# Lacadame/DiffSci

Hardware: AMD Instinct MI355X
Metric: samples/sec (50-step Karras Heun), PUNetG 64ch 128x128 (higher is better)
Workload: dtype f32 (3x3 convs: fp16 hi+lo split, 3 fp16 MFMA products, fp32 accumulate); 1 GPU; PUNetG 64-base-ch, 1x128x128 fields, batch 64 per GPU, 50-step Heun deterministic sampler (99 network evaluations); global_batch=64, parallelism=dp1 (batch shards, all-gather of samples), world_size=1, backend=none (one process), hipgraph=True

## Files before the change

diffsci_amd/_native.py:

```python
import ctypes
import os
from ctypes import POINTER, Structure, c_char_p, c_float, c_int, c_longlong, c_size_t, c_uint32, c_uint64, c_void_p

_HERE = os.path.dirname(os.path.abspath(__file__))
LIB_PATH = os.environ.get("DIFFSCI_HIP_LIB") or os.path.join(_HERE, "_lib", "libdiffsci_hip.so")

ABI_VERSION = 4
DS_IN_NETWORK, DS_IN_SCORE, DS_IN_DRIFT, DS_IN_FLOW = 0, 1, 2, 3
DS_LOAD_PLAIN, DS_LOAD_MAXPOOL2, DS_LOAD_UPSAMPLE2, DS_LOAD_AVGPOOL2 = 0, 1, 2, 3
DS_PAD_CIRCULAR = 16
DS_PAD_ZERO_H, DS_PAD_ZERO_W, DS_PAD_ZERO_D = 64, 128, 0x10000
DS_RES1_UPSAMPLED = 32
DS_PC_RAW, DS_PC_IMAGES = 1, 2
DS_SI_BLEND, DS_SI_RENOISE = 1, 2
DS_DDPM_CLASSICAL, DS_DDPM_GENERALIZED, DS_DDPM_FORWARD = 0, 1, 2
DS_DDPM_NOISE_NONE, DS_DDPM_NOISE_EPS, DS_DDPM_NOISE_PHILOX = 0, 4, 8


class EvalCoef(Structure):
    _fields_ = [("c_out", c_float), ("c_skip", c_float), ("sigma_sq", c_float),
                ("neg_mult", c_float), ("neg_lang", c_float), ("guidance", c_float),
                ("one_minus_guidance", c_float), ("input_kind", c_int), ("stochastic", c_int),
                ("scaled", c_int), ("scale", c_float), ("scale_mult", c_float), ("next_scale", c_float), ("xin_copies", c_int),
                ("nonfinite", c_void_p)]
# ... 64 lines not shown
    "ds_inorm_silu_images_supported": (c_int, [c_int, c_int]),
    "ds_inorm_silu_images": (c_int, [_P, _P, _P, _P, c_int, c_int, c_int, c_int, c_float, c_int, _P]),
    "ds_conv2d_h3_img": (c_int, [_P, _P, _P, c_int, _P, _P, c_int, _P, _P, c_int, c_int, c_int, c_int, c_int, c_int, _P, _P, _P]),
    "ds_gnorm1_apply_images": (c_int, [_P, _P, _P, _P, _P, _P, _P, c_int, c_int, c_int, c_int, c_int, c_int, c_int, _P]),
    "ds_volume_stat_tiles": (c_int, [c_int, c_size_t]),
    "ds_volume_to_slices_act": (c_int, [_P, _P, _P, c_int, c_int, c_int, c_size_t, c_int, _P]),
    "ds_wrap_pad_slices": (c_int, [_P, c_int, c_int, c_int, c_size_t, _P]),
    "ds_slices_to_volume_stats": (c_int, [_P, _P, _P, _P, _P, c_int, c_int, c_int, c_size_t, c_int, _P]),
    "ds_slice_tables": (c_int, [_P, _P, _P, _P, c_int, c_int, c_int, c_int, c_longlong, c_float, c_int, c_int, _P]),
    "ds_avgpool3d": (c_int, [_P, _P, c_int, c_int, c_int, c_int, _P]),
    "ds_upsample3d": (c_int, [_P, _P, c_int, c_int, c_int, c_int, _P]),
    "ds_avgpool3d_f": (c_int, [_P, _P, c_int, c_int, c_int, c_int, c_int, _P]),
    "ds_upsample_f": (c_int, [_P, _P, c_int, c_int, c_int, c_int, c_int, c_int, _P]),
    "ds_maxpool_f": (c_int, [_P, _P, c_int, c_int, c_int, c_int, c_int, c_int, _P]),
    "ds_cornerpool_f": (c_int, [_P, _P, _P, _P, c_int, c_int, c_int, c_int, c_int, c_int, c_int, c_int, c_int, _P]),
    "ds_conv1x1_h3_packed_bytes": (c_size_t, [c_int, c_int]),
    "ds_conv1x1_h3_pack_weights": (c_int, [_P, _P, c_int, c_int, c_int, _P]),
    "ds_conv1x1_h3": (c_int, [_P, _P, _P, c_int, _P, _P, c_int, _P, _P, c_int, c_int, c_int, c_int, c_int, c_int, _P, _P, _P, c_int, _P]),
    "ds_attention": (c_int, [_P, _P, c_int, c_int, c_int, _P]),
    "ds_attention_generic": (c_int, [_P, _P, c_int, c_int, c_int, _P]),
    "ds_attention_h3": (c_int, [_P, _P, c_int, c_int, c_int, _P, _P, _P]),
    "ds_attention_h3_workspace_bytes": (c_size_t, [c_int, c_int, c_int]),
    "ds_attention_h3_ws": (c_int, [_P, _P, _P, c_int, c_int, c_int, _P, _P, _P]),
    "ds_attention_h3_heads_workspace_bytes": (c_size_t, [c_int, c_int, c_int, c_int]),
    "ds_attention_h3_heads": (c_int, [_P, _P, _P, c_int, c_int, c_int, c_int, _P, _P, _P]),
    "ds_attention_heads_generic": (c_int, [_P, _P, c_int, c_int, c_int, c_int, _P]),
    "ds_token_l2_normalize": (c_int, [_P, c_int, c_int, c_int, c_int, c_int, c_float, c_float, _P]),
    "ds_linear": (c_int, [_P, _P, _P, _P, c_int, c_int, c_int, c_int, _P]),
    "ds_fourier_features": (c_int, [_P, _P, _P, _P, c_int, c_int, c_int, _P]),
    "ds_fourier_channels": (c_int, [_P, _P, _P, c_int, c_int, c_int, c_size_t, _P]),
    "ds_gnorm1_workspace_bytes": (c_size_t, [c_int]),
    "ds_gnorm1_stats": (c_int, [_P, _P, _P, c_int, c_int, c_int, c_float, c_int, _P]),
    "ds_groupnorm_stats": (c_int, [_P, _P, _P, c_int, c_int, c_int, c_int, c_float, _P]),
    "ds_groupnorm_apply": (c_int, [_P, _P, _P, _P, _P, c_int, c_int, c_int, c_int, c_int, _P, _P]),
    "ds_groupnorm_stats_tiles": (c_int, [_P, _P, c_int, c_int, c_int, c_int, c_longlong, c_float, _P]),
    "ds_groupnorm_table": (c_int, [_P, _P, _P, _P, _P, c_int, c_int, c_int, c_int, c_longlong, c_float, _P]),
    "ds_gnorm1_apply": (c_int, [_P, _P, _P, _P, _P, _P, _P, c_int, c_int, c_int, c_int, c_int, c_int, c_int, _P]),
    "ds_gnorm1_apply_poolf": (c_int, [_P, _P, _P, _P, _P, _P, _P, c_int, c_int, c_int, c_int, c_int, c_int, c_int, _P]),
    "ds_concat2": (c_int, [_P, _P, _P, c_int, c_size_t, c_size_t, _P]),
    "ds_add_act": (c_int, [_P, _P, _P, c_int, c_int, c_int, c_int, _P]),
    "ds_mask_blend": (c_int, [_P, _P, _P, _P, c_size_t, c_int, _P]),
    "ds_axpby": (c_int, [_P, _P, c_float, _P, c_float, c_size_t, _P]),
    "ds_div_scalar": (c_int, [_P, _P, c_float, c_size_t, _P]),
    "ds_batchnorm_eval": (c_int, [_P, _P, _P, _P, _P, _P, c_float, c_float, c_int, c_int, c_int, c_int, c_size_t, _P]),
    "ds_lerp_stack": (c_int, [_P, _P, _P, c_int, c_size_t, _P]),
    "ds_add": (c_int, [_P, _P, _P, c_size_t, _P]),
# ... 67 lines not shown
```

diffsci_amd/csrc/ds_attn3h.hip:

```cpp
#include <cstdlib>

#include "ds_common.h"
#include "ds_conv_epilogue.h"
#include "ds_h3_common.h"

namespace {

using ds::f32x4;
using ds::wave_max;
using ds_epi::f32x16;
using ds_h3::f16x8;
using ds_h3::split2;
using ds_h3::u32x4;
typedef unsigned u32x2 __attribute__((ext_vector_type(2)));

constexpr int NT = 256;
constexpr int KB = 32;
constexpr float RESCALE_T = 8.0f;

constexpr float LOG2E = 1.44269504088896341f;

__device__ __forceinline__ f16x8 as_f16x8(u32x4 v) { return __builtin_bit_cast(f16x8, v); }

template <int ET, bool IMG, bool MH>
__global__ __launch_bounds__(NT) void k_attn3h(float* out, const float* __restrict__ qkv, const u32x4* __restrict__ kimg,
                                               const u32x4* __restrict__ vimg, int L, int heads, int nb, float scale, float thr,
                                               const unsigned* in_amax, unsigned* out_amax) {
  constexpr int E = 32 * ET;
  constexpr int NDG = E / 8;
  constexpr int NS = E / 16;
  constexpr int KITEMS = NDG * KB;
  constexpr int KI = (KITEMS + NT - 1) / NT;
  constexpr int VITEMS = E * 4;
  constexpr int VI = (VITEMS + NT - 1) / NT;
  extern __shared__ __attribute__((aligned(16))) unsigned char smem[];
  constexpr int KVEC = 2 * NDG * KB;
  constexpr int VVEC = 2 * 4 * E;
  u32x4* Kbuf = reinterpret_cast<u32x4*>(smem);
  u32x4* Vbuf = Kbuf + 2 * KVEC;
  const int tid = threadIdx.x, lane = tid & 63;
  const int wv = __builtin_amdgcn_readfirstlane(tid >> 6);
  const int li = lane & 31, lh = lane >> 5;
  unsigned qblk, b_u;
  {
    const unsigned nx = gridDim.x;
    const unsigned id = blockIdx.x + nx * blockIdx.y;
    const unsigned total = nx * gridDim.y;
    const unsigned per = total >> 3, rem = total & 7u;
    const unsigned xcd = id & 7u, k = id >> 3;
    const unsigned logical = xcd * per + (xcd < rem ? xcd : rem) + k;
    qblk = logical % nx;
    b_u = logical / nx;
  }
  const int row = (int)b_u;
  const int b = MH ? row / heads : row, h = MH ? row - b * heads : 0;
  const int Etot = MH ? E * heads : E;
  const int B = MH ? nb : (int)gridDim.y;
  const int q0_raw = ((int)qblk * 4 + wv) * 32;
  const bool active = q0_raw < L;
  const int q0 = active ? q0_raw : L - 32;
  const float* Qt = qkv + ((size_t)b * 3 * Etot + (size_t)h * E) * L;
  const float* Kt = Qt + (size_t)Etot * L;
  const float* Vt = Kt + (size_t)Etot * L;
  const int ak = ds_epi::act_exponent_of(ds_epi::act_bits(in_amax, b), -60, 60);
  const int av = ds_epi::act_exponent_of(ds_epi::act_bits(in_amax, B + b), -120, 120);
  const float a_in = ds_epi::pow2f(ak), v_in = ds_epi::pow2f(av);
  const float s_un = ds_epi::pow2f(-2 * ak), o_un = ds_epi::pow2f(-av);
  scale = ds_epi::mul_pow2(scale, ak);

  u32x4 qh[NS], ql[NS];
#pragma unroll
  for (int s = 0; s < NS; ++s) {
    float v[8];
#pragma unroll
    for (int k = 0; k < 8; ++k)
      v[k] = Qt[(size_t)(16 * s + 8 * lh + k) * L + q0 + li] * scale;
#pragma unroll
    for (int k = 0; k < 4; ++k) {
      unsigned h, l;
      split2(v[2 * k], v[2 * k + 1], h, l);
      qh[s][k] = h; ql[s][k] = l;
    }
  }

  f32x16 O[ET];
#pragma unroll
  for (int t = 0; t < ET; ++t)
#pragma unroll
    for (int r = 0; r < 16; ++r) O[t][r] = 0.f;
  float m_run = -INFINITY, l_run = 0.f;

// ... 271 lines not shown
    if (IMG) asm volatile("s_waitcnt vmcnt(0)" ::: "memory");
    __syncthreads();
  }
  }
  float amax = 0.f;
  if (active) {
    const float inv = (1.0f / l_run) * o_un;
    float* ob = out + ((size_t)b * Etot + (size_t)h * E) * L;
#pragma unroll
    for (int t = 0; t < ET; ++t)
#pragma unroll
      for (int r = 0; r < 16; ++r) {
        const int d = 32 * t + (r & 3) + 8 * (r >> 2) + 4 * lh;
        const float o = O[t][r] * inv;
        ob[(size_t)d * L + q0 + li] = o;
        amax = fmaxf(amax, __builtin_fabsf(o));
      }
  }
  if (out_amax) ds::wave_commit_max_always(out_amax + b, amax);
}

template <int ET, bool MH>
__global__ __launch_bounds__(NT) void k_attn_images(u32x4* __restrict__ kimg, u32x4* __restrict__ vimg,
                                                   const float* __restrict__ qkv, int L, int heads, int nb,
                                                   const unsigned* in_amax) {
  constexpr int E = 32 * ET, NDG = E / 8;
  constexpr int KITEMS = NDG * KB, VITEMS = E * 4;
  const int tid = threadIdx.x, kb = blockIdx.x, row = blockIdx.y, nkb = L / KB;
  const int b = MH ? row / heads : row, h = MH ? row - b * heads : 0;
  const int Etot = MH ? E * heads : E;
  const int B = MH ? nb : (int)gridDim.y;
  const float a_in = ds_epi::pow2f(ds_epi::act_exponent_of(ds_epi::act_bits(in_amax, b), -60, 60));
  const float v_in = ds_epi::pow2f(ds_epi::act_exponent_of(ds_epi::act_bits(in_amax, B + b), -120, 120));
  const float* Kt = qkv + (((size_t)b * 3 + 1) * Etot + (size_t)h * E) * L + (size_t)kb * KB;
  const float* Vt = Kt + (size_t)Etot * L;
  u32x4* Kd = kimg + ((size_t)row * nkb + kb) * (2 * KITEMS);
  u32x4* Vd = vimg + ((size_t)row * nkb + kb) * (2 * VITEMS);
  for (int e = tid; e < KITEMS; e += NT) {
    const int dg = e / KB, key = e % KB;
    u32x4 h, l;
#pragma unroll
    for (int k = 0; k < 4; ++k) {
      unsigned a, c;
      split2(Kt[(size_t)(8 * dg + 2 * k) * L + key] * a_in, Kt[(size_t)(8 * dg + 2 * k + 1) * L + key] * a_in, a, c);
      h[k] = a; l[k] = c;
    }
    Kd[e] = h;
    Kd[KITEMS + e] = l;
  }
  for (int e = tid; e < VITEMS; e += NT) {
    const int d = e >> 2, kg = e & 3;
    const float* p = Vt + (size_t)d * L + 8 * kg;
    const f32x4 v0 = *reinterpret_cast<const f32x4*>(p) * v_in, v1 = *reinterpret_cast<const f32x4*>(p + 4) * v_in;
    u32x4 h, l;
    unsigned a, c;
    split2(v0[0], v0[1], a, c); h[0] = a; l[0] = c;
    split2(v0[2], v0[3], a, c); h[1] = a; l[1] = c;
    split2(v1[0], v1[1], a, c); h[2] = a; l[2] = c;
    split2(v1[2], v1[3], a, c); h[3] = a; l[3] = c;
    Vd[kg * E + d] = h;
    Vd[VITEMS + kg * E + d] = l;
  }
}

template <int ET, bool IMG, bool MH>
int launch_attn3h(float* out, const float* qkv, void* workspace, int B, int heads, int L, float scale, const unsigned* in_amax,
                  unsigned* out_amax, hipStream_t s) {
  constexpr int E = 32 * ET;
  const size_t lds = (size_t)2 * (2 * (E / 8) * KB + 2 * 4 * E) * 16;
  if (lds > 48 * 1024) {
    const int rc = ds::ensure_dynamic_lds<&k_attn3h<ET, IMG, MH>>((int)lds, "hipFuncSetAttribute(attn3h)");
    if (rc != DS_OK) return rc;
  }
  const int rows = B * heads;
  u32x4* kimg = nullptr;
  u32x4* vimg = nullptr;
  if (IMG) {
    kimg = reinterpret_cast<u32x4*>(workspace);
    vimg = kimg + (size_t)rows * L * (E / 4);
    hipLaunchKernelGGL((k_attn_images<ET, MH>), dim3(L / KB, rows), dim3(NT), 0, s, kimg, vimg, qkv, L, heads, B, in_amax);
    DS_CHECK_LAUNCH("ds_attention_h3 (images)");
  }
  dim3 g((L + 127) / 128, rows);
  hipLaunchKernelGGL((k_attn3h<ET, IMG, MH>), g, dim3(NT), lds, s, out, qkv, kimg, vimg, L, heads, B, scale, RESCALE_T, in_amax,
                     out_amax);
  DS_CHECK_LAUNCH("ds_attention_h3");
  return DS_OK;
}

template <bool IMG>
int attention_h3(float* out, const float* qkv, void* workspace, int B, int E, int L, const unsigned* in_amax, unsigned* out_amax,
                 void* stream) {
  DS_REQUIRE(out && qkv, DS_ERR_NULL, "ds_attention_h3: NULL pointer");
  DS_REQUIRE(B >= 0 && E > 0 && L > 0, DS_ERR_SHAPE, "ds_attention_h3: bad shape B=%d E=%d L=%d", B, E, L);
  DS_REQUIRE(L % 32 == 0, DS_ERR_UNSUPPORTED, "ds_attention_h3: L=%d must be a multiple of 32", L);
  DS_REQUIRE(B < 65536 && L / 32 < 65536 * 32, DS_ERR_SHAPE, "ds_attention_h3: B=%d exceeds grid.y", B);
  DS_REQUIRE((reinterpret_cast<uintptr_t>(qkv) & 15u) == 0, DS_ERR_SHAPE, "ds_attention_h3: qkv must be 16-byte aligned");
  DS_REQUIRE(!IMG || (workspace && (reinterpret_cast<uintptr_t>(workspace) & 15u) == 0), DS_ERR_NULL,
             "ds_attention_h3_ws: a 16-byte aligned workspace of ds_attention_h3_workspace_bytes(B, E, L) bytes is required");
  if (B == 0) return DS_OK;
  const float scale = (float)sqrt(1.0 / (double)E);
  hipStream_t s = ds::as_stream(stream);
  switch (E) {
    case 32: return launch_attn3h<1, IMG, false>(out, qkv, workspace, B, 1, L, scale, in_amax, out_amax, s);
    case 64: return launch_attn3h<2, IMG, false>(out, qkv, workspace, B, 1, L, scale, in_amax, out_amax, s);
    case 128: return launch_attn3h<4, IMG, false>(out, qkv, workspace, B, 1, L, scale, in_amax, out_amax, s);
    case 256: return launch_attn3h<8, IMG, false>(out, qkv, workspace, B, 1, L, scale, in_amax, out_amax, s);
    default:
      ds::set_error("ds_attention_h3: E=%d unsupported (32, 64, 128, 256)", E);
      return DS_ERR_UNSUPPORTED;
  }
}

bool mfma_head_width(int d) { return d == 32 || d == 64 || d == 128 || d == 256; }

__global__ __launch_bounds__(64) void k_attn_heads_generic(float* out, const float* __restrict__ qkv, int d, int heads, int L,
                                                           float scale) {
  extern __shared__ float sm[];
  float* qs = sm;
  float* ps = sm + d;
  const int q = blockIdx.x, row = blockIdx.y, lane = threadIdx.x;
  const int b = row / heads, h = row - b * heads, Etot = d * heads;
  const float* Qt = qkv + ((size_t)b * 3 * Etot + (size_t)h * d) * L;
  const float* Kt = Qt + (size_t)Etot * L;
  const float* Vt = Kt + (size_t)Etot * L;
  for (int c = lane; c < d; c += 64) qs[c] = Qt[(size_t)c * L + q] * scale;
  __syncthreads();
  float mx = -INFINITY;
  for (int k = lane; k < L; k += 64) {
    float sc = 0.f;
    for (int c = 0; c < d; ++c) sc = fmaf(qs[c], Kt[(size_t)c * L + k], sc);
    ps[k] = sc;
    mx = fmaxf(mx, sc);
  }
// ... 29 lines not shown
  const float scale = (float)sqrt(1.0 / (double)d);
  hipLaunchKernelGGL(k_attn_heads_generic, dim3(L, B * heads), dim3(64), lds, s, out, qkv, d, heads, L, scale);
  DS_CHECK_LAUNCH("ds_attention_heads_generic");
  return DS_OK;
}

}

extern "C" int ds_attention_h3(float* out, const float* qkv, int B, int E, int L, const unsigned* in_amax, unsigned* out_amax,
                               void* stream) {
  return attention_h3<false>(out, qkv, nullptr, B, E, L, in_amax, out_amax, stream);
}

extern "C" size_t ds_attention_h3_workspace_bytes(int B, int E, int L) {
  if (B <= 0 || E <= 0 || L <= 0) return 0;
  return (size_t)B * L * E * 8;
}

extern "C" int ds_attention_h3_ws(float* out, const float* qkv, void* workspace, int B, int E, int L, const unsigned* in_amax,
                                  unsigned* out_amax, void* stream) {
  return attention_h3<true>(out, qkv, workspace, B, E, L, in_amax, out_amax, stream);
}

extern "C" size_t ds_attention_h3_heads_workspace_bytes(int B, int E, int heads, int L) {
  if (B <= 0 || E <= 0 || L <= 0 || heads <= 0 || E % heads || !mfma_head_width(E / heads) || L % 32) return 0;
  return (size_t)B * L * E * 8;
}

extern "C" int ds_attention_h3_heads(float* out, const float* qkv, void* workspace, int B, int E, int heads, int L,
                                     const unsigned* in_amax, unsigned* out_amax, void* stream) {
  DS_REQUIRE(out && qkv, DS_ERR_NULL, "ds_attention_h3_heads: NULL pointer");
  DS_REQUIRE(B >= 0 && E > 0 && L > 0 && heads > 0, DS_ERR_SHAPE, "ds_attention_h3_heads: bad shape B=%d E=%d heads=%d L=%d",
             B, E, heads, L);
  DS_REQUIRE(E % heads == 0, DS_ERR_SHAPE, "ds_attention_h3_heads: E=%d is not a multiple of heads=%d", E, heads);
  DS_REQUIRE((size_t)B * heads < 65536, DS_ERR_SHAPE, "ds_attention_h3_heads: B*heads=%lld exceeds grid.y", (long long)B * heads);
  if (heads == 1) {
    if (workspace) return attention_h3<true>(out, qkv, workspace, B, E, L, in_amax, out_amax, stream);
    return attention_h3<false>(out, qkv, nullptr, B, E, L, in_amax, out_amax, stream);
  }
  if (B == 0) return DS_OK;
  const int d = E / heads;
  const float scale = (float)sqrt(1.0 / (double)d);
  hipStream_t s = ds::as_stream(stream);
  if (!mfma_head_width(d) || L % 32) {
    DS_REQUIRE(out_amax == nullptr, DS_ERR_UNSUPPORTED,
               "ds_attention_h3_heads: out_amax needs a head width in {32, 64, 128, 256} and L a multiple of 32 (reduce with "
               "ds_absmax_rows instead)");
    return heads_generic(out, qkv, B, E, heads, L, s);
  }
  DS_REQUIRE((reinterpret_cast<uintptr_t>(qkv) & 15u) == 0, DS_ERR_SHAPE, "ds_attention_h3_heads: qkv must be 16-byte aligned");
  DS_REQUIRE(!workspace || (reinterpret_cast<uintptr_t>(workspace) & 15u) == 0, DS_ERR_SHAPE,
             "ds_attention_h3_heads: the workspace must be 16-byte aligned");
  const bool img = workspace != nullptr;
  switch (d) {
    case 32: return img ? launch_attn3h<1, true, true>(out, qkv, workspace, B, heads, L, scale, in_amax, out_amax, s)
                        : launch_attn3h<1, false, true>(out, qkv, nullptr, B, heads, L, scale, in_amax, out_amax, s);
    case 64: return img ? launch_attn3h<2, true, true>(out, qkv, workspace, B, heads, L, scale, in_amax, out_amax, s)
                        : launch_attn3h<2, false, true>(out, qkv, nullptr, B, heads, L, scale, in_amax, out_amax, s);
    case 128: return img ? launch_attn3h<4, true, true>(out, qkv, workspace, B, heads, L, scale, in_amax, out_amax, s)
                         : launch_attn3h<4, false, true>(out, qkv, nullptr, B, heads, L, scale, in_amax, out_amax, s);
    default: return img ? launch_attn3h<8, true, true>(out, qkv, workspace, B, heads, L, scale, in_amax, out_amax, s)
                        : launch_attn3h<8, false, true>(out, qkv, nullptr, B, heads, L, scale, in_amax, out_amax, s);
  }
}

extern "C" int ds_attention_heads_generic(float* out, const float* qkv, int B, int E, int heads, int L, void* stream) {
  DS_REQUIRE(out && qkv, DS_ERR_NULL, "ds_attention_heads_generic: NULL pointer");
  DS_REQUIRE(B >= 0 && E > 0 && L > 0 && heads > 0, DS_ERR_SHAPE, "ds_attention_heads_generic: bad shape B=%d E=%d heads=%d L=%d",
             B, E, heads, L);
  DS_REQUIRE(E % heads == 0, DS_ERR_SHAPE, "ds_attention_heads_generic: E=%d is not a multiple of heads=%d", E, heads);
  DS_REQUIRE((size_t)B * heads < 65536, DS_ERR_SHAPE, "ds_attention_heads_generic: B*heads=%lld exceeds grid.y",
             (long long)B * heads);
  return heads_generic(out, qkv, B, E, heads, L, ds::as_stream(stream));
}
```

diffsci_amd/models/karras/engine.py:

```python
import torch

from ... import ops
from ..._native import DS_IN_NETWORK, DS_IN_SCORE
from ..nets import precision
from ..nets.runtime import tensor_version
from .steptable import StepTable


class ScoreFnSource:
    input_kind = DS_IN_SCORE
    wants_xin = False
    xin_copies = 1
    guidance = 1.0

    def __init__(self, score_fn, batch, like):
        self.score_fn = score_fn
        self.batch = batch
        self.like = like
        self._ones = torch.ones(batch, dtype=torch.float32, device=like.device)

    def prepare(self, table: StepTable):
        pass

    def evaluate(self, state, xin, row, index, slot):
# ... 19 lines not shown
    return ("object", repr(type(y)), id(y))


def clone_condition(y):
    if isinstance(y, dict):
        return {k: clone_condition(v) for k, v in y.items()}
    if isinstance(y, (list, tuple)):
        return type(y)(clone_condition(v) for v in y)
    return y.clone() if torch.is_tensor(y) else y


def copy_condition(dst, src):
    if isinstance(dst, dict):
        for k in dst:
            copy_condition(dst[k], src[k])
    elif isinstance(dst, (list, tuple)):
        for d, v in zip(dst, src):
            copy_condition(d, v)
    elif torch.is_tensor(dst):
        dst.copy_(src)


MODEL_SWITCHES = ("conv_precision", "fuse_norm", "fuse_max_cot", "direct_out", "upsample_parity", "norm_images", "tile_stats_norms",
                  "exact_input_layer", "capturable", "pool_route", "circular_axes")


def _tree_slots(model):
    mods = list(model.modules())
    shape = tuple((d, len(d)) for m in mods for d in (m._modules, m._parameters, m._buffers))
    children = tuple((m._modules, name, c) for m in mods for name, c in m._modules.items())
    params = tuple((m._parameters, name) for m in mods for name, p in m._parameters.items() if p is not None) + \
        tuple((m._buffers, name) for m in mods for name, p in m._buffers.items() if p is not None)
    return shape, children, params


def model_signature(model):
    slots = model.__dict__.get("_signature_slots")
    if slots is not None:
        shape, children, params = slots
        if not (all(len(d) == n for d, n in shape) and all(d.get(name) is c for d, name, c in children)):
            slots = None
    if slots is None:
        slots = model.__dict__["_signature_slots"] = _tree_slots(model)
    out = []
    for d, name in slots[2]:
        p = d[name]
        out.append((p.data_ptr(), tensor_version(p)) if p is not None else None)
# ... 413 lines not shown
```

diffsci_amd/models/nets/punetg.py:

```python
import math
import os
from typing import Any

import torch

from ... import ops
from ..._native import DS_LOAD_MAXPOOL2, DS_LOAD_UPSAMPLE2
from . import commonlayers, precision, runtime
from .punetg_config import PUNetGConfig, scale_factor
from .runtime import AmaxArena, Workspace, _amax_kw, require_eval, shift_rows, weights_signature

POOL_ROUTES = ("loader", "pass", "epilogue")
POOL_ROUTE_DEFAULT = "epilogue"


class _AffineHolder(torch.nn.Module):

    def __init__(self, C, affine=True):
        super().__init__()
        self.weight = torch.nn.Parameter(torch.ones(C)) if affine else None
        self.bias = torch.nn.Parameter(torch.zeros(C)) if affine else None


NORM_KINDS = {"GroupLN": 0, "GroupRMS": 1, "GroupPix": 3}
# ... 198 lines not shown
        mc = config.model_channels
        self.time_projection = _Fourier(mc, config.time_projection_scale)
        self.conditional_embedding = conditional_embedding
        self.cond_drop = (_ConditionDrop(config.cond_drop, mc, config.cond_drop_learnable)
                          if config.cond_drop is not None and config.cond_drop > 0 else None)
        self.circular_axes = (config.convolution_type == "circular",) * config.dimension
        self.mp = config.convolution_type == "mp"
        self.cosine_attn = config.attn_type == "cosine"
        self.inhouse_attn = self.mp or self.cosine_attn
        norms = (config.first_resblock_norm, config.second_resblock_norm)
        self.norm_kinds = tuple(NORM_KINDS.get(n, 2) for n in norms)
        dim = self.dim = config.dimension
        self.convin, self.convout = self.make_convin_and_convout()
        self.downward_blocks, self.downsamplers = self.make_downward_blocks()
        self.upward_blocks, self.upsamplers = self.make_upward_blocks()
        self.before_block, self.after_block = self.make_non_attn_bottom_blocks()
        self.attn_resnet_block, self.attn_block = self.make_attn_bottom_blocks()
        self.conv_precision = "fp16x3"
        self.auto_precision = True
        self.fuse_norm = True
        self.fuse_max_cot = 2
        self.pool_route = os.environ.get("DIFFSCI_POOL_ROUTE", POOL_ROUTE_DEFAULT)
        self.norm_images = os.environ.get("DIFFSCI_NORM_IMAGES", "1") != "0"
        self._packed = None
        self._packed_sig = None
        self._ws = Workspace()
        self._am = None
        self._window_cache = {}
        self.exact_input_layer = False

    def drop_caches(self):
        super().drop_caches()
        self.__dict__.pop("_tb_packed", None)
        self.__dict__.pop("_tb_packed_sig", None)
        self._ws, self._am, self._window_cache = Workspace(), None, {}

    def choose_conv_cls(self):
        if self.config.dimension not in (2, 3):
            raise NotImplementedError("1D convolution not implemented yet") if self.config.dimension == 1 \
                else ValueError(f"Invalid dimension {self.config.dimension}")
        kind, dim = self.config.convolution_type, self.config.dimension

        def conv_cls(in_channels, out_channels, kernel_size, bias=True, **_):
            return make_conv(in_channels, out_channels, kernel_size, kind, bias, dim)
        return conv_cls

    def make_convin_and_convout(self):
        c = self.config
        conv_cls = self.choose_conv_cls()
        cin = c.input_channels + (0 if c.bias else 1)
        if c.in_embedding:
            convin = _FourierInput(cin, c.model_channels, c.input_projection_scale)
        else:
            convin = conv_cls(cin, c.model_channels, c.in_out_kernel_size, bias=bool(c.bias))
        convout = conv_cls(c.model_channels, c.output_channels, c.in_out_kernel_size, bias=bool(c.bias))
        return convin, convout

# ... 565 lines not shown
                xa = xa2
        if nattn == 0:
            xa = ops.add(a[0], a[0], out=ws.take(a[0].shape, dev)), None, None
        give(a)
        a = chain(self.after_block, xa, rest)
        for lv, blocks in enumerate(self.upward_blocks):
            skip = skips.pop()
            a2 = d.up(self.upsamplers[lv], a, skip, blocks[0] if len(blocks) else None)
            give(a)
            ws.give(skip)
            a = chain(blocks, a2, self.upsamplers[lv + 1] if lv + 1 < nup else self.convout)
        y = d.out(a, out)
        give(a)
        return y

    def _attention(self, att, x, pk, ws, res2=None, tile_stats=None, in_amax=None, out_amax=None):
        m = att.mhattn
        in_bias = None if self.inhouse_attn else m.in_proj_bias
        out_bias = None if self.inhouse_attn else m.out_proj.bias
        am = self._am if self.conv_precision == "fp16x3" else None
        own = None
        if am is None and self.conv_precision == "fp16x3":
            own = am = AmaxArena(ws, x.shape[0], x.device)
        y = runtime.attention(x, pk[(id(att), "in")], in_bias, pk[(id(att), "out")], out_bias, E=x.shape[1],
                              heads=getattr(m, "num_heads", 1), precision=self.conv_precision, ws=ws, am=am, in_amax=in_amax,
                              out_amax=out_amax, res1=x if self.config.attn_residual else None, res2=res2, tile_stats=tile_stats,
                              cosine=self.cosine_attn)
        if own is not None:
            own.release()
        return y


def _shift_source(shifts, row, B):
    if isinstance(shifts, _FieldShifts):
        return lambda: shifts
    it = iter(shifts)
    return lambda: shift_rows(next(it), row, B)


class _Fields:

    def __init__(self, net, x, shifts, row):
        if net.pool_route not in POOL_ROUTES:
            raise ValueError(f"pool_route {net.pool_route!r}; choose from {POOL_ROUTES}")
        self.net, self.pk, self.ws = net, net.packed_weights(), net._ws
        self.B, self.dev = x.shape[0], x.device
        self.sh = _shift_source(shifts, row, self.B)
        self.h3 = net.conv_precision == "fp16x3"
        lazy = self.h3 and not isinstance(net.convin, _FourierInput) and not net.exact_input_layer
        self.am = net._am = AmaxArena(self.ws, self.B, self.dev, zero=not lazy) if self.h3 else None
        self.direct_out = net._out_is_direct(net.convout)
        self.pool = None

# ... 269 lines not shown
```

diffsci_amd/models/nets/runtime.py:

```python
import math

import torch

from ... import ops
from . import precision


def require_eval(net, *rates):
    if net.training and any(r for r in rates if r):
        raise NotImplementedError("dropout / cond_dropout / cond_drop > 0 in training mode are outside the HIP sampling "
                                  "path: call .eval() (the reference samples under eval() too)")


class Workspace:

    def __init__(self):
        self.free = {}
        self.frozen = False
        self.bytes = 0

    def take(self, shape, device):
        key = (tuple(shape), str(device))
        lst = self.free.get(key)
        if lst:
# ... 75 lines not shown
    if row is not None:
        if s.dim() == 3:
            if s.shape[1] != B:
                raise ValueError("time embedding batch does not match x")
            return s[row]
        return s[row:row + 1]
    if s.shape[0] not in (1, B):
        raise ValueError("time embedding batch does not match x")
    return s


def guarded_forward(net, run, *inputs):
    out = run(*inputs)
    if precision.needs_escalation(net, out, inputs[0]):
        precision.escalate(net)
        out = run(*inputs)
    return out


def _amax_kw(pack, **kw):
    return kw if pack.kind == "fp16x3" else {}


def attention(x4, w_in, b_in, w_out, b_out, *, E, heads, precision, ws=None, am=None, in_amax=None, out_amax=None,
              res1=None, res2=None, tile_stats=None, cosine=False, attn_out=None):
    B, _, Hh, Ww = x4.shape
    L = Hh * Ww
    dev = x4.device

    def take(shape):
        return torch.empty(shape, dtype=torch.float32, device=dev) if ws is None else ws.take(shape, dev)

    def give(t):
        if ws is not None and t is not None:
            ws.give(t)

    a_qkv = a_o = None
    if w_in.kind == "fp16x3":
        a_qkv, a_o = (ops.amax_new(2 * B, dev), ops.amax_new(B, dev)) if am is None else (am.rows(2), am.row())
        if in_amax is None and am is not None:
            in_amax = am.of(x4)
    split = 2 * E if E % 32 == 0 else 0
    direct = split > 0 and not cosine
    qkv = ops.conv(x4, w_in, bias=b_in, out=take((B, 3 * E, Hh, Ww)),
                   **_amax_kw(w_in, in_amax=in_amax, out_amax=a_qkv if direct else None, amax_split=split if direct else 0))
    if cosine:
        ops.token_l2_normalize(qkv.view(B, 3 * E, L), 0, E, eps=1e-8, gain=math.sqrt(E))
        ops.token_l2_normalize(qkv.view(B, 3 * E, L), E, E, eps=1e-8, gain=1.0)
    if a_qkv is not None and not direct:
        ops.absmax_rows(qkv[:, :2 * E], out=a_qkv[:B])
        ops.absmax_rows(qkv[:, 2 * E:], out=a_qkv[B:])
    nws = ops.attention_workspace_floats(B, E, L, precision, heads=heads)
    aws = take((nws,)) if nws else None
    o = ops.attention(qkv.view(B, 3 * E, L), E, out=take((B, E, L)) if attn_out is None else attn_out, precision=precision,
                      workspace=aws, heads=heads, **_amax_kw(w_in, in_amax=a_qkv, out_amax=a_o))
    give(aws)
    y = ops.conv(o.view(B, E, Hh, Ww), w_out, bias=b_out, res1=res1, res2=res2, tile_stats=tile_stats, out=take(x4.shape),
                 **_amax_kw(w_out, in_amax=a_o, out_amax=out_amax))
    give(qkv)
# ... 3 lines not shown
```

diffsci_amd/ops.py:

```python
import ctypes
import gc

import torch

from . import _native as N
from ._native import EvalCoef


def _off_device(t):
    if not t.is_cuda:
        return "host"
    return None if t.device.index == torch.cuda.current_device() else "other"


def require_device(t, what="tensor"):
    if not isinstance(t, torch.Tensor):
        raise TypeError(f"{what} must be a torch.Tensor")
    off = _off_device(t)
    if not off and t.dtype == torch.float32:
        return
    if off == "host":
        raise RuntimeError(
            f"{what} lives on {t.device}: diffsci_amd computes only on an AMD GPU through "
            "libdiffsci_hip.so (there is no CPU path; move the module and inputs to 'cuda').")
# ... 1555 lines not shown
        elif L % 32 != 0 or E not in (32, 64, 128, 256, 384, 512):
            N.check(lib.ds_attention_generic(_p(out), _p(qkv), B, E, L, _stream()), "ds_attention_generic")
        else:
            N.check(lib.ds_attention(_p(out), _p(qkv), B, E, L, _stream()), "ds_attention")
        if out_amax is not None:
            absmax_rows(out, B, out=out_amax)
        return out
    if in_amax is None:
        in_amax = amax_new(2 * B, qkv.device)
        absmax_rows(qkv[:, :2 * E], out=in_amax[:B])
        absmax_rows(qkv[:, 2 * E:], out=in_amax[B:])
    pin, pout = (None if in_amax is NORMALISED else _pi(in_amax, 2 * B, "in_amax")), _pi(out_amax, B, "out_amax")
    need = attention_workspace_floats(B, E, L, precision, heads)
    pws = _p(_workspace(workspace, 4 * need, qkv, "attention workspace too small"), "workspace") if need else None
    if heads > 1:
        N.check(lib.ds_attention_h3_heads(_p(out), _p(qkv), pws, B, E, heads, L, pin, pout, _stream()), "ds_attention_h3_heads")
    elif need:
        N.check(lib.ds_attention_h3_ws(_p(out), _p(qkv), pws, B, E, L, pin, pout, _stream()), "ds_attention_h3_ws")
    else:
        N.check(lib.ds_attention_h3(_p(out), _p(qkv), B, E, L, pin, pout, _stream()), "ds_attention_h3")
    return out


def linear(x, w, b=None, act=0, out=None):
    M, K = x.shape
    Nn, K2 = w.shape
    if K != K2:
        raise ValueError("linear: inner dimensions differ")
    _entries(b, Nn, "linear: b must have N={} entries", Nn)
    out = _out(out, (M, Nn), x)
    N.check(N.lib().ds_linear(_p(out), _p(x), _p(w), _p(b), M, K, Nn, act, _stream()), "ds_linear")
    return out


def fourier_features(t, W, add=None, out=None):
    M, half = t.numel(), W.numel()
    add_rows = 0
    if add is not None:
        if add.dim() < 1 or add.shape[-1] != 2 * half:
            raise ValueError(f"fourier_features: add must hold rows of {2 * half} entries; got {tuple(add.shape)}")
        add = add.reshape(-1, 2 * half)
        add_rows = add.shape[0]
    out = _out(out, (M, 2 * half), t)
    N.check(N.lib().ds_fourier_features(_p(out), _p(t), _p(W), _p(add), add_rows, M, half, _stream()),
            "ds_fourier_features")
    return out
# ... 283 lines not shown
```

include/diffsci_hip.h:

```cpp
#ifndef DIFFSCI_HIP_H
#define DIFFSCI_HIP_H

#include <stddef.h>
#include <stdint.h>

#ifdef __cplusplus
extern "C" {
#endif

typedef enum ds_status {
  DS_OK = 0,
  DS_ERR_SHAPE = -1,
  DS_ERR_NULL = -2,
  DS_ERR_HIP = -3,
  DS_ERR_UNSUPPORTED = -4
} ds_status;

int ds_version(void);
const char* ds_last_error(void);
int ds_device_info(int* cu_count, int* lds_bytes_per_cu, char* arch_name, int arch_name_len);

typedef struct ds_eval_coef {
  float c_out;
  float c_skip;
// ... 151 lines not shown

int ds_maxpool_f(float* out, const float* x, int planes, int Di, int Hi, int Wi, int factor, int volume, void* stream);

int ds_cornerpool_f(float* out, const float* x, const float* te, unsigned* out_amax, int B, int C, int Di, int Hi, int Wi,
                    int factor, int volume, int x_batch, int te_batch, void* stream);

size_t ds_conv1x1_h3_packed_bytes(int Cout, int Cin);
int ds_conv1x1_h3_pack_weights(void* packed, const float* w, int Cout, int Cin, int wshift, void* stream);
int ds_conv1x1_h3(float* out, const float* in, const void* w_packed, int wshift, const float* bias,
                  const float* shift, int shift_stride, const float* res1, const float* res2,
                  int B, int Cin, int Cout, int H, int W, int load_mode, float* tile_stats,
                  const unsigned* in_amax, unsigned* out_amax, int amax_split, void* stream);

int ds_attention(float* out, const float* qkv, int B, int E, int L, void* stream);

int ds_attention_generic(float* out, const float* qkv, int B, int E, int L, void* stream);

int ds_token_l2_normalize(float* x, int B, int Ctot, int c0, int C, int L, float eps, float gain, void* stream);

int ds_attention_h3(float* out, const float* qkv, int B, int E, int L, const unsigned* in_amax, unsigned* out_amax, void* stream);
size_t ds_attention_h3_workspace_bytes(int B, int E, int L);
int ds_attention_h3_ws(float* out, const float* qkv, void* workspace, int B, int E, int L, const unsigned* in_amax,
                       unsigned* out_amax, void* stream);
size_t ds_attention_h3_heads_workspace_bytes(int B, int E, int heads, int L);
int ds_attention_h3_heads(float* out, const float* qkv, void* workspace, int B, int E, int heads, int L, const unsigned* in_amax,
                          unsigned* out_amax, void* stream);
int ds_attention_heads_generic(float* out, const float* qkv, int B, int E, int heads, int L, void* stream);

int ds_linear(float* y, const float* x, const float* w, const float* b, int M, int K, int N, int act, void* stream);

int ds_fourier_features(float* out, const float* t, const float* W, const float* add, int add_rows,
                        int M, int half, void* stream);

int ds_fourier_channels(float* out, const float* x, const float* W, int B, int C, int D, size_t HW, void* stream);


size_t ds_gnorm1_workspace_bytes(int B);
int ds_gnorm1_stats(float* stats, void* workspace, const float* x, int B, int C, int HW, float eps, int kind,
                    void* stream);

int ds_groupnorm_stats(float* stats, void* workspace, const float* x, int B, int C, int G, int N, float eps, void* stream);
int ds_groupnorm_apply(float* out, const float* x, const float* stats, const float* w, const float* b, int B, int C, int G, int N,
                       int act, unsigned* out_amax, void* stream);
int ds_groupnorm_stats_tiles(float* stats, const float* tile_stats, int B, int C, int G, int ntiles, long long count, float eps,
                             void* stream);
int ds_groupnorm_table(float* table, const float* tile_stats, const float* stats, const float* w, const float* b, int B, int C,
// ... 113 lines not shown
```

Before: 84.20 samples/s.

## Fold key/value projections into query and output weights for single-head attention

Precomputes M = Wk^T Wq and Wp = Wout Wv (with matching biases) so attention runs on q' = M x and uses the block input x directly as keys and values. This removes the 3E-channel QKV projection, keeping only an E-channel projection, and drops the separate value projection. A new kernel entry point takes separate q/k/v sources with their own strides and amax scales. Folded weights are cached per module, and the changed factorisation may shift fp16-split rounding slightly.

```diff
diff --git a/diffsci_amd/_native.py b/diffsci_amd/_native.py
--- a/diffsci_amd/_native.py
+++ b/diffsci_amd/_native.py
@@ -110,6 +110,7 @@
     "ds_attention_h3": (c_int, [_P, _P, c_int, c_int, c_int, _P, _P, _P]),
     "ds_attention_h3_workspace_bytes": (c_size_t, [c_int, c_int, c_int]),
     "ds_attention_h3_ws": (c_int, [_P, _P, _P, c_int, c_int, c_int, _P, _P, _P]),
+    "ds_attention_h3_xkv": (c_int, [_P, _P, _P, _P, c_int, c_int, c_int, _P, _P, _P, _P, _P, c_int]),
     "ds_attention_h3_heads_workspace_bytes": (c_size_t, [c_int, c_int, c_int, c_int]),
     "ds_attention_h3_heads": (c_int, [_P, _P, _P, c_int, c_int, c_int, c_int, _P, _P, _P]),
     "ds_attention_heads_generic": (c_int, [_P, _P, c_int, c_int, c_int, c_int, _P]),
diff --git a/diffsci_amd/csrc/ds_attn3h.hip b/diffsci_amd/csrc/ds_attn3h.hip
--- a/diffsci_amd/csrc/ds_attn3h.hip
+++ b/diffsci_amd/csrc/ds_attn3h.hip
@@ -23,9 +23,10 @@
 __device__ __forceinline__ f16x8 as_f16x8(u32x4 v) { return __builtin_bit_cast(f16x8, v); }
 
 template <int ET, bool IMG, bool MH>
-__global__ __launch_bounds__(NT) void k_attn3h(float* out, const float* __restrict__ qkv, const u32x4* __restrict__ kimg,
-                                               const u32x4* __restrict__ vimg, int L, int heads, int nb, float scale, float thr,
-                                               const unsigned* in_amax, unsigned* out_amax) {
+__global__ __launch_bounds__(NT) void k_attn3h(float* out, const float* __restrict__ q, size_t q_bs,
+                                               const u32x4* __restrict__ kimg, const u32x4* __restrict__ vimg, int L, int heads,
+                                               float scale, float thr, const unsigned* q_amax, const unsigned* k_amax,
+                                               const unsigned* v_amax, unsigned* out_amax) {
   constexpr int E = 32 * ET;
   constexpr int NDG = E / 8;
   constexpr int NS = E / 16;
@@ -55,18 +56,19 @@
   const int row = (int)b_u;
   const int b = MH ? row / heads : row, h = MH ? row - b * heads : 0;
   const int Etot = MH ? E * heads : E;
-  const int B = MH ? nb : (int)gridDim.y;
   const int q0_raw = ((int)qblk * 4 + wv) * 32;
   const bool active = q0_raw < L;
   const int q0 = active ? q0_raw : L - 32;
-  const float* Qt = qkv + ((size_t)b * 3 * Etot + (size_t)h * E) * L;
+  const float* Qt = q + (size_t)b * q_bs + (size_t)h * E * L;
   const float* Kt = Qt + (size_t)Etot * L;
   const float* Vt = Kt + (size_t)Etot * L;
-  const int ak = ds_epi::act_exponent_of(ds_epi::act_bits(in_amax, b), -60, 60);
-  const int av = ds_epi::act_exponent_of(ds_epi::act_bits(in_amax, B + b), -120, 120);
+  const unsigned q_bits = ds_epi::act_bits(q_amax, b), k_bits = ds_epi::act_bits(k_amax, b), v_bits = ds_epi::act_bits(v_amax, b);
+  const int aq = ds_epi::act_exponent_of(q_bits, -60, 60);
+  const int ak = ds_epi::act_exponent_of(k_bits, -60, 60);
+  const int av = ds_epi::act_exponent_of(v_bits, -120, 120);
   const float a_in = ds_epi::pow2f(ak), v_in = ds_epi::pow2f(av);
-  const float s_un = ds_epi::pow2f(-2 * ak), o_un = ds_epi::pow2f(-av);
-  scale = ds_epi::mul_pow2(scale, ak);
+  const float s_un = ds_epi::pow2f(-(aq + ak)), o_un = ds_epi::pow2f(-av);
+  scale = ds_epi::mul_pow2(scale, aq);
 
   u32x4 qh[NS], ql[NS];
 #pragma unroll
@@ -384,18 +386,16 @@
 
 template <int ET, bool MH>
 __global__ __launch_bounds__(NT) void k_attn_images(u32x4* __restrict__ kimg, u32x4* __restrict__ vimg,
-                                                   const float* __restrict__ qkv, int L, int heads, int nb,
-                                                   const unsigned* in_amax) {
+                                                   const float* __restrict__ ksrc, size_t k_bs, const float* __restrict__ vsrc,
+                                                   size_t v_bs, int L, int heads, const unsigned* k_amax, const unsigned* v_amax) {
   constexpr int E = 32 * ET, NDG = E / 8;
   constexpr int KITEMS = NDG * KB, VITEMS = E * 4;
   const int tid = threadIdx.x, kb = blockIdx.x, row = blockIdx.y, nkb = L / KB;
   const int b = MH ? row / heads : row, h = MH ? row - b * heads : 0;
-  const int Etot = MH ? E * heads : E;
-  const int B = MH ? nb : (int)gridDim.y;
-  const float a_in = ds_epi::pow2f(ds_epi::act_exponent_of(ds_epi::act_bits(in_amax, b), -60, 60));
-  const float v_in = ds_epi::pow2f(ds_epi::act_exponent_of(ds_epi::act_bits(in_amax, B + b), -120, 120));
-  const float* Kt = qkv + (((size_t)b * 3 + 1) * Etot + (size_t)h * E) * L + (size_t)kb * KB;
-  const float* Vt = Kt + (size_t)Etot * L;
+  const float a_in = ds_epi::pow2f(ds_epi::act_exponent_of(ds_epi::act_bits(k_amax, b), -60, 60));
+  const float v_in = ds_epi::pow2f(ds_epi::act_exponent_of(ds_epi::act_bits(v_amax, b), -120, 120));
+  const float* Kt = ksrc + (size_t)b * k_bs + (size_t)h * E * L + (size_t)kb * KB;
+  const float* Vt = vsrc + (size_t)b * v_bs + (size_t)h * E * L + (size_t)kb * KB;
   u32x4* Kd = kimg + ((size_t)row * nkb + kb) * (2 * KITEMS);
   u32x4* Vd = vimg + ((size_t)row * nkb + kb) * (2 * VITEMS);
   for (int e = tid; e < KITEMS; e += NT) {
@@ -425,9 +425,19 @@
   }
 }
 
+struct AttnSrc {
+  const float *q, *k, *v;
+  size_t q_bs, k_bs, v_bs;
+  const unsigned *q_amax, *k_amax, *v_amax;
+};
+AttnSrc qkv_src(const float* qkv, int B, int Etot, int L, const unsigned* in_amax) {
+  const size_t third = (size_t)Etot * L;
+  return AttnSrc{qkv, qkv + third, qkv + 2 * third, 3 * third, 3 * third, 3 * third, in_amax, in_amax, in_amax ? in_amax + B : nullptr};
+}
+
 template <int ET, bool IMG, bool MH>
-int launch_attn3h(float* out, const float* qkv, void* workspace, int B, int heads, int L, float scale, const unsigned* in_amax,
-                  unsigned* out_amax, hipStream_t s) {
+int launch_attn3h(float* out, const AttnSrc& a, void* workspace, int B, int heads, int L, float scale, unsigned* out_amax,
+                  hipStream_t s) {
   constexpr int E = 32 * ET;
   const size_t lds = (size_t)2 * (2 * (E / 8) * KB + 2 * 4 * E) * 16;
   if (lds > 48 * 1024) {
@@ -440,14 +450,29 @@
   if (IMG) {
     kimg = reinterpret_cast<u32x4*>(workspace);
     vimg = kimg + (size_t)rows * L * (E / 4);
-    hipLaunchKernelGGL((k_attn_images<ET, MH>), dim3(L / KB, rows), dim3(NT), 0, s, kimg, vimg, qkv, L, heads, B, in_amax);
+    hipLaunchKernelGGL((k_attn_images<ET, MH>), dim3(L / KB, rows), dim3(NT), 0, s, kimg, vimg, a.k, a.k_bs, a.v, a.v_bs, L, heads,
+                       a.k_amax, a.v_amax);
     DS_CHECK_LAUNCH("ds_attention_h3 (images)");
   }
   dim3 g((L + 127) / 128, rows);
-  hipLaunchKernelGGL((k_attn3h<ET, IMG, MH>), g, dim3(NT), lds, s, out, qkv, kimg, vimg, L, heads, B, scale, RESCALE_T, in_amax,
-                     out_amax);
+  hipLaunchKernelGGL((k_attn3h<ET, IMG, MH>), g, dim3(NT), lds, s, out, a.q, a.q_bs, kimg, vimg, L, heads, scale, RESCALE_T,
+                     a.q_amax, a.k_amax, a.v_amax, out_amax);
   DS_CHECK_LAUNCH("ds_attention_h3");
   return DS_OK;
+}
+
+template <bool IMG>
+int attention_h3_src(float* out, const AttnSrc& a, void* workspace, int B, int E, int L, unsigned* out_amax, hipStream_t s) {
+  const float scale = (float)sqrt(1.0 / (double)E);
+  switch (E) {
+    case 32: return launch_attn3h<1, IMG, false>(out, a, workspace, B, 1, L, scale, out_amax, s);
+    case 64: return launch_attn3h<2, IMG, false>(out, a, workspace, B, 1, L, scale, out_amax, s);
+    case 128: return launch_attn3h<4, IMG, false>(out, a, workspace, B, 1, L, scale, out_amax, s);
+    case 256: return launch_attn3h<8, IMG, false>(out, a, workspace, B, 1, L, scale, out_amax, s);
+    default:
+      ds::set_error("ds_attention_h3: E=%d unsupported (32, 64, 128, 256)", E);
+      return DS_ERR_UNSUPPORTED;
+  }
 }
 
 template <bool IMG>
@@ -461,17 +486,7 @@
   DS_REQUIRE(!IMG || (workspace && (reinterpret_cast<uintptr_t>(workspace) & 15u) == 0), DS_ERR_NULL,
              "ds_attention_h3_ws: a 16-byte aligned workspace of ds_attention_h3_workspace_bytes(B, E, L) bytes is required");
   if (B == 0) return DS_OK;
-  const float scale = (float)sqrt(1.0 / (double)E);
-  hipStream_t s = ds::as_stream(stream);
-  switch (E) {
-    case 32: return launch_attn3h<1, IMG, false>(out, qkv, workspace, B, 1, L, scale, in_amax, out_amax, s);
-    case 64: return launch_attn3h<2, IMG, false>(out, qkv, workspace, B, 1, L, scale, in_amax, out_amax, s);
-    case 128: return launch_attn3h<4, IMG, false>(out, qkv, workspace, B, 1, L, scale, in_amax, out_amax, s);
-    case 256: return launch_attn3h<8, IMG, false>(out, qkv, workspace, B, 1, L, scale, in_amax, out_amax, s);
-    default:
-      ds::set_error("ds_attention_h3: E=%d unsupported (32, 64, 128, 256)", E);
-      return DS_ERR_UNSUPPORTED;
-  }
+  return attention_h3_src<IMG>(out, qkv_src(qkv, B, E, L, in_amax), workspace, B, E, L, out_amax, ds::as_stream(stream));
 }
 
 bool mfma_head_width(int d) { return d == 32 || d == 64 || d == 128 || d == 256; }
@@ -547,6 +562,24 @@
   return attention_h3<true>(out, qkv, workspace, B, E, L, in_amax, out_amax, stream);
 }
 
+extern "C" int ds_attention_h3_xkv(float* out, const float* q, const float* x, void* workspace, int B, int E, int L,
+                                   const unsigned* q_amax, const unsigned* k_amax, const unsigned* v_amax, unsigned* out_amax,
+                                   void* stream, int flags) {
+  DS_REQUIRE(out && q && x, DS_ERR_NULL, "ds_attention_h3_xkv: NULL pointer");
+  DS_REQUIRE(flags == 0, DS_ERR_UNSUPPORTED, "ds_attention_h3_xkv: flags=%d must be 0", flags);
+  DS_REQUIRE(B >= 0 && E > 0 && L > 0, DS_ERR_SHAPE, "ds_attention_h3_xkv: bad shape B=%d E=%d L=%d", B, E, L);
+  DS_REQUIRE(L % 32 == 0, DS_ERR_UNSUPPORTED, "ds_attention_h3_xkv: L=%d must be a multiple of 32", L);
+  DS_REQUIRE(B < 65536 && L / 32 < 65536 * 32, DS_ERR_SHAPE, "ds_attention_h3_xkv: B=%d exceeds grid.y", B);
+  DS_REQUIRE(((reinterpret_cast<uintptr_t>(q) | reinterpret_cast<uintptr_t>(x)) & 15u) == 0, DS_ERR_SHAPE,
+             "ds_attention_h3_xkv: q and x must be 16-byte aligned");
+  DS_REQUIRE(workspace && (reinterpret_cast<uintptr_t>(workspace) & 15u) == 0, DS_ERR_NULL,
+             "ds_attention_h3_xkv: a 16-byte aligned workspace of ds_attention_h3_workspace_bytes(B, E, L) bytes is required");
+  if (B == 0) return DS_OK;
+  const size_t bs = (size_t)E * L;
+  return attention_h3_src<true>(out, AttnSrc{q, x, x, bs, bs, bs, q_amax, k_amax, v_amax}, workspace, B, E, L, out_amax,
+                                ds::as_stream(stream));
+}
+
 extern "C" size_t ds_attention_h3_heads_workspace_bytes(int B, int E, int heads, int L) {
   if (B <= 0 || E <= 0 || L <= 0 || heads <= 0 || E % heads || !mfma_head_width(E / heads) || L % 32) return 0;
   return (size_t)B * L * E * 8;
@@ -577,15 +610,16 @@
   DS_REQUIRE(!workspace || (reinterpret_cast<uintptr_t>(workspace) & 15u) == 0, DS_ERR_SHAPE,
              "ds_attention_h3_heads: the workspace must be 16-byte aligned");
   const bool img = workspace != nullptr;
+  const AttnSrc a = qkv_src(qkv, B, E, L, in_amax);
   switch (d) {
-    case 32: return img ? launch_attn3h<1, true, true>(out, qkv, workspace, B, heads, L, scale, in_amax, out_amax, s)
-                        : launch_attn3h<1, false, true>(out, qkv, nullptr, B, heads, L, scale, in_amax, out_amax, s);
-    case 64: return img ? launch_attn3h<2, true, true>(out, qkv, workspace, B, heads, L, scale, in_amax, out_amax, s)
-                        : launch_attn3h<2, false, true>(out, qkv, nullptr, B, heads, L, scale, in_amax, out_amax, s);
-    case 128: return img ? launch_attn3h<4, true, true>(out, qkv, workspace, B, heads, L, scale, in_amax, out_amax, s)
-                         : launch_attn3h<4, false, true>(out, qkv, nullptr, B, heads, L, scale, in_amax, out_amax, s);
-    default: return img ? launch_attn3h<8, true, true>(out, qkv, workspace, B, heads, L, scale, in_amax, out_amax, s)
-                        : launch_attn3h<8, false, true>(out, qkv, nullptr, B, heads, L, scale, in_amax, out_amax, s);
+    case 32: return img ? launch_attn3h<1, true, true>(out, a, workspace, B, heads, L, scale, out_amax, s)
+                        : launch_attn3h<1, false, true>(out, a, nullptr, B, heads, L, scale, out_amax, s);
+    case 64: return img ? launch_attn3h<2, true, true>(out, a, workspace, B, heads, L, scale, out_amax, s)
+                        : launch_attn3h<2, false, true>(out, a, nullptr, B, heads, L, scale, out_amax, s);
+    case 128: return img ? launch_attn3h<4, true, true>(out, a, workspace, B, heads, L, scale, out_amax, s)
+                         : launch_attn3h<4, false, true>(out, a, nullptr, B, heads, L, scale, out_amax, s);
+    default: return img ? launch_attn3h<8, true, true>(out, a, workspace, B, heads, L, scale, out_amax, s)
+                        : launch_attn3h<8, false, true>(out, a, nullptr, B, heads, L, scale, out_amax, s);
   }
 }
 
diff --git a/diffsci_amd/models/karras/engine.py b/diffsci_amd/models/karras/engine.py
--- a/diffsci_amd/models/karras/engine.py
+++ b/diffsci_amd/models/karras/engine.py
@@ -65,7 +65,7 @@
 
 
 MODEL_SWITCHES = ("conv_precision", "fuse_norm", "fuse_max_cot", "direct_out", "upsample_parity", "norm_images", "tile_stats_norms",
-                  "exact_input_layer", "capturable", "pool_route", "circular_axes")
+                  "exact_input_layer", "capturable", "pool_route", "circular_axes", "attn_fold")
 
 
 def _tree_slots(model):
diff --git a/diffsci_amd/models/nets/punetg.py b/diffsci_amd/models/nets/punetg.py
--- a/diffsci_amd/models/nets/punetg.py
+++ b/diffsci_amd/models/nets/punetg.py
@@ -244,6 +244,7 @@
         self.fuse_max_cot = 2
         self.pool_route = os.environ.get("DIFFSCI_POOL_ROUTE", POOL_ROUTE_DEFAULT)
         self.norm_images = os.environ.get("DIFFSCI_NORM_IMAGES", "1") != "0"
+        self.attn_fold = os.environ.get("DIFFSCI_ATTN_FOLD", "1") != "0"
         self._packed = None
         self._packed_sig = None
         self._ws = Workspace()
@@ -255,6 +256,7 @@
         super().drop_caches()
         self.__dict__.pop("_tb_packed", None)
         self.__dict__.pop("_tb_packed_sig", None)
+        self.__dict__.pop("_attn_folded", None)
         self._ws, self._am, self._window_cache = Workspace(), None, {}
 
     def choose_conv_cls(self):
@@ -866,13 +868,43 @@
         own = None
         if am is None and self.conv_precision == "fp16x3":
             own = am = AmaxArena(ws, x.shape[0], x.device)
-        y = runtime.attention(x, pk[(id(att), "in")], in_bias, pk[(id(att), "out")], out_bias, E=x.shape[1],
-                              heads=getattr(m, "num_heads", 1), precision=self.conv_precision, ws=ws, am=am, in_amax=in_amax,
+        E, heads = x.shape[1], getattr(m, "num_heads", 1)
+        folded = None
+        if self.attn_fold:
+            probe = runtime.FoldedAttention(pk[(id(att), "in")], None, pk[(id(att), "out")], None)
+            if runtime.attention_folds(probe, E, x.shape[2] * x.shape[3], heads, self.conv_precision, self.cosine_attn):
+                folded = self._folded_attention(att)
+        y = runtime.attention(x, pk[(id(att), "in")], in_bias, pk[(id(att), "out")], out_bias, E=E,
+                              heads=heads, precision=self.conv_precision, ws=ws, am=am, in_amax=in_amax,
                               out_amax=out_amax, res1=x if self.config.attn_residual else None, res2=res2, tile_stats=tile_stats,
-                              cosine=self.cosine_attn)
+                              cosine=self.cosine_attn, folded=folded)
         if own is not None:
             own.release()
         return y
+
+    def _folded_attention(self, att):
+        m = att.mhattn
+        if self.inhouse_attn:
+            tracked = [m.q_proj_matrix, m.k_proj_matrix, m.v_proj_matrix, m.o_proj_matrix]
+        else:
+            tracked = [t for t in (m.in_proj_weight, m.out_proj.weight, m.in_proj_bias, m.out_proj.bias) if t is not None]
+        sig = weights_signature(tracked, self.conv_precision)
+        cache = self.__dict__.setdefault("_attn_folded", {})
+        hit = cache.get(id(att))
+        if hit is not None and hit[0] == sig:
+            return hit[1]
+        with torch.no_grad():
+            if self.inhouse_attn:
+                (w_in, w_out), b_in, b_out = m.projection_weights(), None, None
+            else:
+                w_in, w_out, b_in, b_out = m.in_proj_weight, m.out_proj.weight, m.in_proj_bias, m.out_proj.bias
+            E = m.embed_dim
+            M, c, Wp, bp = runtime.fold_attention_weights(w_in, b_in, w_out, b_out)
+            f32 = lambda t: None if t is None else t.float().contiguous()
+            folded = runtime.FoldedAttention(ops.pack_conv(f32(M).reshape(E, E, 1, 1), "fp16x3"), f32(c),
+                                             ops.pack_conv(f32(Wp).reshape(E, E, 1, 1), "fp16x3"), f32(bp))
+        cache[id(att)] = (sig, folded)
+        return folded
 
 
 def _shift_source(shifts, row, B):
diff --git a/diffsci_amd/models/nets/runtime.py b/diffsci_amd/models/nets/runtime.py
--- a/diffsci_amd/models/nets/runtime.py
+++ b/diffsci_amd/models/nets/runtime.py
@@ -121,8 +121,34 @@
     return kw if pack.kind == "fp16x3" else {}
 
 
+class FoldedAttention:
+    __slots__ = ("w_q", "b_q", "w_out", "b_out")
+
+    def __init__(self, w_q, b_q, w_out, b_out):
+        self.w_q, self.b_q, self.w_out, self.b_out = w_q, b_q, w_out, b_out
+
+
+def fold_attention_weights(w_in, b_in, w_out, b_out):
+    E = w_out.shape[0]
+    w_in, w_out = w_in.detach().double().reshape(3 * E, E), w_out.detach().double().reshape(E, E)
+    wq, wk, wv = w_in[:E], w_in[E:2 * E], w_in[2 * E:]
+    M, Wp = wk.t() @ wq, w_out @ wv
+    c = bp = None
+    if b_in is not None:
+        b_in = b_in.detach().double()
+        c, bp = wk.t() @ b_in[:E], w_out @ b_in[2 * E:]
+    if b_out is not None:
+        bp = b_out.detach().double() + (0 if bp is None else bp)
+    return M, c, Wp, bp
+
+
+def attention_folds(folded, E, L, heads, precision, cosine):
+    return (folded is not None and folded.w_q.kind == "fp16x3" and folded.w_out.kind == "fp16x3" and heads == 1 and not cosine
+            and ops._attention_uses_images(E, L, precision))
+
+
 def attention(x4, w_in, b_in, w_out, b_out, *, E, heads, precision, ws=None, am=None, in_amax=None, out_amax=None,
-              res1=None, res2=None, tile_stats=None, cosine=False, attn_out=None):
+              res1=None, res2=None, tile_stats=None, cosine=False, attn_out=None, folded=None):
     B, _, Hh, Ww = x4.shape
     L = Hh * Ww
     dev = x4.device
@@ -134,6 +160,20 @@
         if ws is not None and t is not None:
             ws.give(t)
 
+    if attention_folds(folded, E, L, heads, precision, cosine):
+        a_q, a_o = (ops.amax_new(B, dev), ops.amax_new(B, dev)) if am is None else (am.row(), am.row())
+        if in_amax is None:
+            in_amax = ops.absmax_rows(x4, B) if am is None else am.of(x4)
+        q = ops.conv(x4, folded.w_q, bias=folded.b_q, out=take((B, E, Hh, Ww)), in_amax=in_amax, out_amax=a_q)
+        aws = take((ops.attention_workspace_floats(B, E, L, precision),))
+        o = ops.attention_xkv(q.view(B, E, L), x4.view(B, E, L), E, out=take((B, E, L)) if attn_out is None else attn_out,
+                              workspace=aws, q_amax=a_q, x_amax=in_amax, out_amax=a_o)
+        give(aws)
+        y = ops.conv(o.view(B, E, Hh, Ww), folded.w_out, bias=folded.b_out, res1=res1, res2=res2, tile_stats=tile_stats,
+                     out=take(x4.shape), in_amax=a_o, out_amax=out_amax)
+        give(q)
+        give(None if attn_out is not None else o)
+        return y
     a_qkv = a_o = None
     if w_in.kind == "fp16x3":
         a_qkv, a_o = (ops.amax_new(2 * B, dev), ops.amax_new(B, dev)) if am is None else (am.rows(2), am.row())
diff --git a/diffsci_amd/ops.py b/diffsci_amd/ops.py
--- a/diffsci_amd/ops.py
+++ b/diffsci_amd/ops.py
@@ -1601,6 +1601,32 @@
     return out
 
 
+def attention_xkv(q, x, E, out=None, workspace=None, q_amax=None, x_amax=None, out_amax=None):
+    B, Eq, L = q.shape
+    if Eq != E or tuple(x.shape) != (B, E, L):
+        raise ValueError(f"attention_xkv: q and x must be [B, E={E}, L]; got {tuple(q.shape)} and {tuple(x.shape)}")
+    if not _attention_uses_images(E, L, "fp16x3"):
+        raise ValueError(f"attention_xkv: E={E}, L={L} is outside the image form (E in 32, 64, 128, 256; L % 32 == 0; "
+                         f"L >= {ATTN_IMAGES_MIN_L}, or {ATTN_IMAGES_MIN_L_WIDE} at E = 256)")
+    out = _out(out, (B, E, L), q)
+    pq, px = _p(q, "q"), _p(x, "x")
+    if B == 0:
+        return out
+    if (pq | px) & 15:
+        raise ValueError("attention_xkv: q and x must be 16-byte aligned")
+    if q_amax is None:
+        q_amax = absmax_rows(q, B)
+    if x_amax is None:
+        x_amax = absmax_rows(x, B)
+    paq = None if q_amax is NORMALISED else _pi(q_amax, B, "q_amax")
+    pax = None if x_amax is NORMALISED else _pi(x_amax, B, "x_amax")
+    need = N.lib().ds_attention_h3_workspace_bytes(B, E, L)
+    pws = _p(_workspace(workspace, need, q, "attention workspace too small"), "workspace")
+    N.check(N.lib().ds_attention_h3_xkv(_p(out), pq, px, pws, B, E, L, paq, pax, pax, _pi(out_amax, B, "out_amax"), _stream(), 0),
+            "ds_attention_h3_xkv")
+    return out
+
+
 def linear(x, w, b=None, act=0, out=None):
     M, K = x.shape
     Nn, K2 = w.shape
diff --git a/include/diffsci_hip.h b/include/diffsci_hip.h
--- a/include/diffsci_hip.h
+++ b/include/diffsci_hip.h
@@ -197,6 +197,8 @@
 size_t ds_attention_h3_workspace_bytes(int B, int E, int L);
 int ds_attention_h3_ws(float* out, const float* qkv, void* workspace, int B, int E, int L, const unsigned* in_amax,
                        unsigned* out_amax, void* stream);
+int ds_attention_h3_xkv(float* out, const float* q, const float* x, void* workspace, int B, int E, int L, const unsigned* q_amax,
+                        const unsigned* k_amax, const unsigned* v_amax, unsigned* out_amax, void* stream, int flags);
 size_t ds_attention_h3_heads_workspace_bytes(int B, int E, int heads, int L);
 int ds_attention_h3_heads(float* out, const float* qkv, void* workspace, int B, int E, int heads, int L, const unsigned* in_amax,
                           unsigned* out_amax, void* stream);
```

New measurement: 85.08 samples/s, median of 6. 1.01x the previous value.
